# Ensembl/WiggleTools

Hardware: AMD Instinct MI355X
Metric: genomic bp/s (whole node) for 'mean' over N BigWig tracks (higher is better)
Workload: dtype f64

## Files before the change

### wiggletools_amd/csrc/wt_core.h

```cpp
#ifndef WT_CORE_H_
#define WT_CORE_H_

#include <stdint.h>
#include <math.h>
#include <type_traits>

#ifdef WT_EMU
#define WT_DEV inline
#define WT_RESTRICT
#else
#include <hip/hip_runtime.h>
#define WT_DEV __device__ __forceinline__
#define WT_RESTRICT __restrict__
#endif

enum {
    WT_OP_SUM = 0, WT_OP_PRODUCT = 1, WT_OP_MEAN = 2, WT_OP_VAR = 3, WT_OP_STDDEV = 4,
    WT_OP_ENTROPY = 5, WT_OP_CV = 6, WT_OP_MIN = 7, WT_OP_MAX = 8, WT_OP_MEDIAN = 9,
    WT_OP_TTEST = 10, WT_OP_MWU = 11,
    WT_OP_MULTIPLEX = 12
};
#define WT_STRICT_SET0 1u
#define WT_STRICT_SET1 2u

#define WT_FLAG_AGG  (1ull << 62)
#define WT_FLAG_PFX  (2ull << 62)
#define WT_VAL_MASK  ((1ull << 62) - 1)

enum { WT_CTR_TICKET = 0, WT_CTR_RUNS = 1, WT_CTR_BP = 2, WT_CTR_INTERVALS = 3, WT_CTR_ERROR = 4,
       WT_CTR_DELTA_BAD = 5 ,
       WT_CTR_PROF = 8 , WT_CTR_N = 16 };
#define WT_ERR_CAPACITY 1ull
#define WT_ERR_LOOKBACK 2ull

struct WtParams {
    const int32_t *start;
    const int32_t *finish;
    const void *value;
    const int64_t *seg_off;
    const double *defaults;
    int32_t n_chrom, n_tracks;
    long long n_total;
    const int32_t *cbase;
    const int32_t *c_nwin;
    const int32_t *c_hi;
    const int64_t *c_first_win;
    int32_t W;
    int32_t logW;
    int32_t n_words;
    int64_t n_windows;
    const int32_t *win_chrom;
    uint32_t *widx;
    int32_t op;
    uint32_t flags;
    int32_t n_set0;
    int32_t pad0;
    unsigned long long *status;
    unsigned long long *counters;
    unsigned long long *debug;
    int64_t capacity;
    int32_t *o_start;
    int32_t *o_finish;
    double *o_value;
    int64_t *chrom_run_off;
    double *o_tile;
    uint8_t *o_inplay;
    int32_t *bad_list;
    long long *bad_goff;
    char *g_scratch;
    long long g_scratch_slab;
    long long g_attr_slab;
    int32_t chunk_tracks;
    int32_t n_chunks;
    int32_t count_segs;
    int32_t spitch;
    int32_t cpitch;
    int32_t off_S, off_cnt, off_segtot, off_U, off_cover, off_E, off_epfx, off_nextw, off_gbase, off_scratch, off_shared;
    int32_t off_acc, off_ev, off_ltv, off_ltc, off_gtv, off_gtc, off_tbase, off_tpfx, off_tfirst, off_dsh;
    int32_t off_qa, off_ltq, off_gtq;
    int32_t delta_q;
    int32_t off_tdef;
    int32_t delta_df;
    int32_t def_emin, def_emax;
    int32_t off_dflt32;
    int32_t off_wcol, off_wcnt, off_woff, off_wtot, off_wbase, off_wgt, off_wncov, off_wfe, off_wdk, off_wguess;
    int32_t walk_S;
    int32_t walk_capp;
    int32_t walk_ov;
    int32_t walk_pair;
    int32_t walk_off_at;
    int32_t walk_mwu;
    int32_t lds_bytes;
    const double *mwu_table;
    int32_t mwu_kmax;
    int32_t delta_ns;
};

struct WtShared {
    long long ticket;
    long long goffset;
    int32_t chrom, w0, w1, emit_hi;
    long long row;
    int32_t next_bp;
    int32_t n_emit;
    unsigned long long bp_sum;
    unsigned long long n_intervals;
    int32_t bad_slot;
};

template <int K>
struct WtLane {
    double res[K];
};

struct WtCtx {
    uint64_t *SC;
    uint16_t *cnt;
    uint32_t *segtot;
    uint64_t *U;
    uint32_t *cover;
    uint64_t *E;
    uint32_t *epfx;
    int16_t *nextw;
    long long *gbase;
    char *scratch;
    char *attr;
    float *dflt32;
    WtShared *sh;
};

WT_DEV void wt_ctx_init(WtCtx &c, const WtParams &P, char *lds) {
    c.SC = (uint64_t *) (lds + P.off_S);
    c.cnt = (uint16_t *) (lds + P.off_cnt);
    c.segtot = (uint32_t *) (lds + P.off_segtot);
    c.U = (uint64_t *) (lds + P.off_U);
    c.cover = (uint32_t *) (lds + P.off_cover);
    c.E = (uint64_t *) (lds + P.off_E);
    c.epfx = (uint32_t *) (lds + P.off_epfx);
    c.nextw = (int16_t *) (lds + P.off_nextw);
// ... 1459 lines not shown
```

### wiggletools_amd/csrc/wt_delta.h

```cpp
#ifndef WT_DELTA_H_
#define WT_DELTA_H_

#define WT_DELTA_K 8
#define WT_DELTA_GROUP 16
#ifndef WT_DELTA_PARK
#define WT_DELTA_PARK 1
#endif
#ifndef WT_DELTA_U
#define WT_DELTA_U 4
#endif
#define WT_DELTA_TILE (64 * WT_DELTA_U)
#ifndef WT_DELTA_COPY2
#define WT_DELTA_COPY2 1
#endif
#ifndef WT_DELTA_ONE_TILE
#define WT_DELTA_ONE_TILE 1
#endif
#define WT_DELTA_TF 2048
#define WT_MAX_DELTA_T 1024
#define WT_DELTA_SQ_T0 768

struct WtDeltaShared {
    long long base_v;
    int32_t base_c;
// ... 145 lines not shown

WT_DEV int wt_delta_find(const uint32_t *tpfx, int nt, uint32_t jj, int i) {
    int lo = i, hi = nt - 1;
    while (lo < hi) {
        const int mid = (lo + hi) >> 1;
        if (jj >= tpfx[mid + 1]) lo = mid + 1; else hi = mid;
    }
    return lo;
}

template <int U = WT_DELTA_U>
WT_DEV void wt_delta_tile(const WtDeltaCtx &d, int nt, uint32_t M, uint32_t tb, int lane, long long (&g)[U]) {
    const uint32_t tile = tb / (64u * U);
    int i = tile < WT_DELTA_TF ? (int) d.tfirst[tile] : wt_delta_find(d.tpfx, nt, tb, 0);
#pragma unroll
    for (int u = 0; u < U; u++) {
        const uint32_t jj = tb + (uint32_t) lane + 64u * (uint32_t) u;
        g[u] = -1;
        if (jj < M) {
            while (jj >= d.tpfx[i + 1]) i++;
            g[u] = d.tbase[i] + 4ll * (long long) jj;
        }
    }
}

template <int U = WT_DELTA_U>
WT_DEV void wt_delta_pass1(const WtParams &P, WtCtx &c, WtDeltaCtx &d, int tid, int nt) {
    const int wave = tid >> 6, lane = tid & 63, nwaves = nt >> 6;
    const uint32_t *val = (const uint32_t *) P.value;
    const uint32_t M = d.tpfx[nt];
    const uint32_t step = (uint32_t) nwaves * (64u * U);
    int emin = 255, emax = 0, bad = 0;
    uint32_t cur[U], nxt[U];
    uint32_t tb = (uint32_t) wave * (64u * U);
    if (tb < M) {
        long long g[U];
        wt_delta_tile<U>(d, nt, M, tb, lane, g);
#pragma unroll
        for (int u = 0; u < U; u++) cur[u] = g[u] >= 0 ? *(const uint32_t *) ((const char *) val + g[u]) : 0u;
    }
    for (; tb < M; tb += step) {
        if (tb + step < M) {
            long long g[U];
            wt_delta_tile<U>(d, nt, M, tb + step, lane, g);
#pragma unroll
            for (int u = 0; u < U; u++) nxt[u] = g[u] >= 0 ? *(const uint32_t *) ((const char *) val + g[u]) : 0u;
        }
#pragma unroll
        for (int u = 0; u < U; u++) {
            const int e = (int) ((cur[u] >> 23) & 0xffu);
            if (e == 0xff) bad = 1;
            if ((cur[u] & 0x7fffffffu) != 0u) {
                const int ee = e ? e : 1;
                emin = ee < emin ? ee : emin;
                emax = ee > emax ? ee : emax;
            }
        }
#pragma unroll
        for (int u = 0; u < U; u++) cur[u] = nxt[u];
    }
    if (emin <= emax) { wt_lds_min32(&d.dsh->emin, emin); wt_lds_max32(&d.dsh->emax, emax); }
    if (bad) wt_lds_max32(&d.dsh->bad, 1);
}

WT_DEV bool wt_delta_verdict(const WtParams &P, const WtDeltaCtx &d, int &emin) {
    int lo = d.dsh->emin, hi = d.dsh->emax;
    if (lo > hi) { lo = 1; hi = 1; }
    emin = lo;
    return !d.dsh->bad && (hi - lo) <= wt_delta_max_span(P.n_tracks);
}

struct WtDeltaRange {
    uint32_t kmax, kmin;
};

WT_DEV long long wt_delta_scaled(uint32_t vb, int scale) {
    const uint32_t e = (vb >> 23) & 0xffu;
    const uint32_t m = (vb & 0x7fffffu) | ((e < 1u ? e : 1u) << 23);
    const int32_t sgn = (int32_t) vb >> 31;
    const int32_t sm = (int32_t) ((m ^ (uint32_t) sgn) - (uint32_t) sgn);
    return (long long) ((unsigned long long) (long long) sm << (((e > 1u ? e : 1u) - (uint32_t) scale) & 63u));
}

template <bool QQ = false, bool DF = false, bool TT = false>
WT_DEV void wt_delta_apply(WtDeltaCtx &d, WtCtx &c, int32_t w0, uint32_t width, int32_t s, int32_t f, uint32_t vb, uint32_t db,
                           int scale, bool ok, int32_t &my_next, WtDeltaRange &R) {
    const uint32_t key = vb & 0x7fffffffu;
    R.kmax = key > R.kmax ? key : R.kmax;
    R.kmin = key - 1u < R.kmin ? key - 1u : R.kmin;
    long long vi = wt_delta_scaled(vb, scale);
    if (DF) vi -= wt_delta_scaled(db, scale);
    const uint32_t po = TT ? db : 0u;
#ifdef WT_EMU
    if (!ok) vi = 0;
#endif
    const uint32_t cs = (uint32_t) (s - w0), cf = (uint32_t) (f - w0);
    if (cs < width && cf < width) {
        wt_lds_add64((unsigned long long *) &d.acc[po + cs], (unsigned long long) vi);
        wt_lds_add32(&d.ev[po + cs], 1u);
        wt_lds_sub64((unsigned long long *) &d.acc[po + cf], (unsigned long long) vi);
        wt_lds_add32(&d.ev[po + cf], 0x10000u);
        if (QQ && vi) {
            unsigned long long a, b;
            wt_delta_square((unsigned long long) (vi < 0 ? -vi : vi), a, b);
            wt_lds_add64(&d.qa[po + cs], a); wt_lds_add64(&d.qb[po + cs], b);
            wt_lds_sub64(&d.qa[po + cf], a); wt_lds_sub64(&d.qb[po + cf], b);
        }
        return;
    }
    const int32_t w1 = w0 + (int32_t) width;
    if (f == w0) { wt_lds_add32(&d.ev[po], 0x00010001u); return; }
    if (s >= w1) { my_next = s < my_next ? s : my_next; return; }
    unsigned long long qa = 0, qb = 0;
    if (QQ && vi) wt_delta_square((unsigned long long) (vi < 0 ? -vi : vi), qa, qb);
    if (s < w0) {
        const bool second = TT && po != 0u;
        wt_lds_add64((unsigned long long *) (second ? &d.dsh->base_v1 : &d.dsh->base_v), (unsigned long long) vi);
        wt_lds_addi32(second ? &d.dsh->base_c1 : &d.dsh->base_c, 1);
        if (QQ && vi) { wt_lds_add64(second ? &d.dsh->base_qa1 : &d.dsh->base_qa, qa); wt_lds_add64(second ? &d.dsh->base_qb1 : &d.dsh->base_qb, qb); }
    } else {
        if (vi) wt_lds_add64((unsigned long long *) &d.acc[po + cs], (unsigned long long) vi);
        wt_lds_add32(&d.ev[po + cs], 1u);
        if (QQ && vi) { wt_lds_add64(&d.qa[po + cs], qa); wt_lds_add64(&d.qb[po + cs], qb); }
    }
    if (f < w1) {
        if (vi) wt_lds_sub64((unsigned long long *) &d.acc[po + cf], (unsigned long long) vi);
        wt_lds_add32(&d.ev[po + cf], 0x10000u);
        if (QQ && vi) { wt_lds_sub64(&d.qa[po + cf], qa); wt_lds_sub64(&d.qb[po + cf], qb); }
    } else {
        my_next = f < my_next ? f : my_next;
    }
}

template <bool DF>
struct WtDeltaPend {
    unsigned long long mask;
    int32_t s, f;
    uint32_t b;
    uint32_t d[DF ? 1 : 1];
};
#ifdef WT_EMU
WT_DEV unsigned long long wt_delta_ballot(bool c) { return c ? 1ull : 0ull; }
WT_DEV bool wt_delta_in_mask(unsigned long long m, int lane) { return m != 0ull; }
#else
WT_DEV unsigned long long wt_delta_ballot(bool c) { return __builtin_amdgcn_ballot_w64(c); }
WT_DEV bool wt_delta_in_mask(unsigned long long m, int lane) { return (m >> lane) & 1ull; }
#endif
template <bool QQ, bool DF, bool TT = false>
WT_DEV void wt_delta_flush(WtDeltaCtx &d, WtCtx &c, WtDeltaPend<DF || TT> &pn, int lane, int32_t w0, uint32_t width, int scale, bool ok,
                           int32_t &my_next) {
    if (wt_delta_in_mask(pn.mask, lane)) {
        WtDeltaRange scrap;
        scrap.kmax = 0u; scrap.kmin = 0xffffffffu;
        wt_delta_apply<QQ, DF, TT>(d, c, w0, width, pn.s, pn.f, pn.b, (DF || TT) ? pn.d[0] : 0u, scale, ok, my_next, scrap);
    }
    pn.mask = 0ull;
}
template <bool QQ, bool DF, bool TT = false>
WT_DEV void wt_delta_apply_or_park(WtDeltaCtx &d, WtCtx &c, WtDeltaPend<DF || TT> &pn, int lane, bool valid, int32_t w0, uint32_t width,
                                   int32_t s, int32_t f, uint32_t vb, uint32_t db, int scale, bool ok, int32_t &my_next, WtDeltaRange &R) {
    const uint32_t rs = (uint32_t) (s - w0), rf = (uint32_t) (f - w0);
    const bool inside = rs < width && rf < width;
    const uint32_t cs = TT ? rs + db : rs, cf = TT ? rf + db : rf;
    if (valid) {
        const uint32_t key = vb & 0x7fffffffu;
        R.kmax = key > R.kmax ? key : R.kmax;
        R.kmin = key - 1u < R.kmin ? key - 1u : R.kmin;
    }
    if (valid && inside) {
        long long vi = wt_delta_scaled(vb, scale);
        if (DF) vi -= wt_delta_scaled(db, scale);
#ifdef WT_EMU
        if (!ok) vi = 0;
#endif
        wt_lds_add64((unsigned long long *) &d.acc[cs], (unsigned long long) vi);
        wt_lds_add32(&d.ev[cs], 1u);
        wt_lds_sub64((unsigned long long *) &d.acc[cf], (unsigned long long) vi);
        wt_lds_add32(&d.ev[cf], 0x10000u);
        if (QQ && vi) {
            unsigned long long a, b;
            wt_delta_square((unsigned long long) (vi < 0 ? -vi : vi), a, b);
            wt_lds_add64(&d.qa[cs], a); wt_lds_add64(&d.qb[cs], b);
            wt_lds_sub64(&d.qa[cf], a); wt_lds_sub64(&d.qb[cf], b);
        }
    }
    const bool park = valid && !inside;
    const unsigned long long pm = wt_delta_ballot(park);
    if (pm & pn.mask) wt_delta_flush<QQ, DF, TT>(d, c, pn, lane, w0, width, scale, ok, my_next);
    pn.s = park ? s : pn.s;
    pn.f = park ? f : pn.f;
    pn.b = park ? vb : pn.b;
    if (DF || TT) pn.d[0] = park ? db : pn.d[0];
    pn.mask |= pm;
}

template <bool DF, int U = WT_DELTA_U>
struct WtDeltaBatch {
    int32_t s[U], f[U];
    uint32_t b[U];
    uint32_t d[DF ? U : 1];
};

template <bool DF, bool TT = false, int U = WT_DELTA_U>
WT_DEV void wt_delta_fetch(const WtParams &P, const WtDeltaCtx &d, int nt, uint32_t M, uint32_t tb, int lane, WtDeltaBatch<DF || TT, U> &B, int c0 = 0) {
    const uint32_t last = (M - 1u) / (64u * U) * (64u * U);
    const uint32_t tbe = tb < last ? tb : last;
    const uint32_t tile = tbe / (64u * U);
    int i = tile < WT_DELTA_TF ? (int) d.tfirst[tile] : wt_delta_find(d.tpfx, nt, tbe, 0);
    uint32_t hi = d.tpfx[i + 1];
    long long dl = d.tbase[i];
    uint32_t db = DF ? d.tdef[i] : 0u;
    if (TT) db = c0 + i >= P.n_set0 ? (uint32_t) P.W : 0u;
#pragma unroll
    for (int u = 0; u < U; u++) {
        uint32_t jj = tbe + (uint32_t) lane + 64u * (uint32_t) u;
        jj = jj < M - 1u ? jj : M - 1u;
        if (jj >= hi) {
            do { i++; hi = d.tpfx[i + 1]; } while (jj >= hi);
            dl = d.tbase[i];
            if (DF) db = d.tdef[i];
            if (TT) db = c0 + i >= P.n_set0 ? (uint32_t) P.W : 0u;
        }
        const long long ob = dl + ((long long) jj << 2);
        B.s[u] = *(const int32_t *) ((const char *) P.start + ob);
        B.f[u] = *(const int32_t *) ((const char *) P.finish + ob);
        B.b[u] = *(const uint32_t *) ((const char *) P.value + ob);
        if (DF || TT) B.d[u] = db;
    }
}


template <bool QQ = false, bool DF = false, bool TT = false, int U = WT_DELTA_U>
WT_DEV void wt_delta_apply_tile(WtDeltaCtx &d, WtCtx &c, const WtDeltaBatch<DF || TT, U> &B, uint32_t tb, uint32_t M, int lane, int32_t w0,
                                uint32_t width, int scale, bool ok, int32_t &my_next, WtDeltaRange &R, WtDeltaPend<DF || TT> &pn) {
    if constexpr (WT_DELTA_PARK == 2 || (WT_DELTA_PARK == 1 && QQ)) {
        if (tb + (64u * U) <= M) {
#pragma unroll
            for (int u = 0; u < U; u++)
                wt_delta_apply_or_park<QQ, DF, TT>(d, c, pn, lane, true, w0, width, B.s[u], B.f[u], B.b[u], (DF || TT) ? B.d[u] : 0u, scale, ok, my_next, R);
        } else {
#pragma unroll
            for (int u = 0; u < U; u++)
                wt_delta_apply_or_park<QQ, DF, TT>(d, c, pn, lane, tb + (uint32_t) lane + 64u * (uint32_t) u < M, w0, width, B.s[u], B.f[u], B.b[u],
                                               (DF || TT) ? B.d[u] : 0u, scale, ok, my_next, R);
        }
    } else {
        if (tb + (64u * U) <= M) {
#pragma unroll
            for (int u = 0; u < U; u++)
                wt_delta_apply<QQ, DF, TT>(d, c, w0, width, B.s[u], B.f[u], B.b[u], (DF || TT) ? B.d[u] : 0u, scale, ok, my_next, R);
        } else {
#pragma unroll
            for (int u = 0; u < U; u++)
                if (tb + (uint32_t) lane + 64u * (uint32_t) u < M)
                    wt_delta_apply<QQ, DF, TT>(d, c, w0, width, B.s[u], B.f[u], B.b[u], (DF || TT) ? B.d[u] : 0u, scale, ok, my_next, R);
        }
    }
}

template <bool QQ = false, bool DF = false, bool TT = false, int U = WT_DELTA_U>
WT_DEV void wt_delta_pass2(const WtParams &P, WtCtx &c, WtDeltaCtx &d, int scale, bool ok, bool collect, bool stats,
                           int tid, int nt, int ntr = 0, int c0 = 0) {
    const int wave = wt_uniform32(tid >> 6), lane = tid & 63, nwaves = nt >> 6;
    const uint32_t M = (uint32_t) wt_uniform32((int32_t) d.tpfx[nt]);
    const int32_t w0 = wt_uniform32(c.sh->w0);
    const uint32_t width = (uint32_t) (wt_uniform32(c.sh->w1) - w0);
    const uint32_t step = (uint32_t) nwaves * (64u * U);
    int32_t my_next = 0x7fffffff;
    WtDeltaRange R;
    R.kmax = 0u; R.kmin = 0xffffffffu;
    if (DF) {
        unsigned long long dsum = (tid < ntr && ok) ? (unsigned long long) wt_delta_scaled(d.tdef[tid], scale) : 0ull;
        dsum = wt_wave_sum_u64(dsum);
        if (dsum && wt_wave_leader(lane)) wt_lds_add64((unsigned long long *) &d.dsh->base_v, dsum);
    }
    uint32_t tb = (uint32_t) wave * (64u * U);
    if (tb < M) {
        WtDeltaBatch<DF || TT, U> A, B;
        WtDeltaPend<DF || TT> pn;
        pn.mask = 0ull; pn.s = 0; pn.f = 0; pn.b = 0u; pn.d[0] = 0u;
        wt_delta_fetch<DF, TT, U>(P, d, nt, M, tb, lane, A, c0);
#if WT_DELTA_ONE_TILE
        if (tb + step >= M) wt_delta_apply_tile<QQ, DF, TT, U>(d, c, A, tb, M, lane, w0, width, scale, ok, my_next, R, pn);
        else
#endif
        for (;;) {
            wt_delta_fetch<DF, TT, U>(P, d, nt, M, tb + step, lane, B, c0);
            wt_delta_apply_tile<QQ, DF, TT, U>(d, c, A, tb, M, lane, w0, width, scale, ok, my_next, R, pn);
            tb += step;
            if (tb >= M) break;
            wt_delta_fetch<DF, TT, U>(P, d, nt, M, tb + step, lane, A, c0);
            wt_delta_apply_tile<QQ, DF, TT, U>(d, c, B, tb, M, lane, w0, width, scale, ok, my_next, R, pn);
            tb += step;
            if (tb >= M) break;
        }
        if (pn.mask) wt_delta_flush<QQ, DF, TT>(d, c, pn, lane, w0, width, scale, ok, my_next);
    }
    my_next = wt_wave_min_i32(my_next);
    if (my_next != 0x7fffffff && wt_wave_leader(lane)) wt_lds_min32(&c.sh->next_bp, my_next);
    if (collect) {
        const uint32_t kmax = wt_wave_max_u32(R.kmax), kmin = wt_wave_min_u32(R.kmin) + 1u;
        if (kmax != 0u && wt_wave_leader(lane)) {
            const int emax = (int) (kmax >> 23), emin = (int) (kmin >> 23);
            wt_lds_min32(&d.dsh->emin, emin ? emin : 1);
            wt_lds_max32(&d.dsh->emax, emax ? emax : 1);
            if (emax == 0xff) wt_lds_max32(&d.dsh->bad, 1);
        }
    }
    if (stats && tid == 0 && M) wt_lds_add64(&c.sh->n_intervals, (unsigned long long) M);
}

WT_DEV int wt_delta_window_verdict(const WtParams &P, const WtDeltaCtx &d, int guess, int &lo, bool &ok) {
    int a = d.dsh->emin, b = d.dsh->emax;
    const bool bad = d.dsh->bad != 0;
    const int R = wt_delta_max_span(P.n_tracks);
    if (a > b) { lo = guess; ok = !bad; return bad ? 0 : 1; }
    lo = a;
    ok = !bad && (b - a) <= R;
    return (!bad && a >= guess && (b - guess) <= R) ? 1 : 0;
}

WT_DEV void wt_delta_mark_bad(const WtParams &P, WtCtx &c, long long k) {
    const unsigned long long slot = wt_glb_add64(&P.counters[WT_CTR_DELTA_BAD], 1ull);
    c.sh->bad_slot = (int32_t) slot;
    if (P.bad_list) P.bad_list[slot] = (int32_t) k;
}
#define WT_BAD_SUB 16
WT_DEV void wt_delta_note_offset(const WtParams &P, WtCtx &c, int lane) {
    if (c.sh->bad_slot >= 0 && P.bad_goff && lane < WT_BAD_SUB)
        P.bad_goff[(long long) c.sh->bad_slot * WT_BAD_SUB + lane] = c.sh->goffset + (long long) c.epfx[(lane * P.n_words) / WT_BAD_SUB];
}

template <bool QQ = false, bool TT = false>
WT_DEV void wt_delta_rezero(const WtParams &P, WtCtx &c, WtDeltaCtx &d, int tid, int nt) {
    const int np = TT ? 2 * P.W : P.W;
    for (int x = tid; x < np; x += nt) { d.acc[x] = 0; d.ev[x] = 0; }
    if constexpr (QQ)
        for (int x = tid; x < np; x += nt) { d.qa[x] = 0; d.qb[x] = 0; }
    if (tid == 0) {
        d.dsh->base_v = 0; d.dsh->base_c = 0;
        if constexpr (QQ) { d.dsh->base_qa = 0; d.dsh->base_qb = 0; }
        if constexpr (TT) { d.dsh->base_v1 = 0; d.dsh->base_c1 = 0; d.dsh->base_qa1 = 0; d.dsh->base_qb1 = 0; }
    }
}

#ifdef WT_EMU
WT_DEV void wt_lds_load8(const uint32_t *p, uint32_t (&v)[WT_DELTA_K]) { for (int k = 0; k < WT_DELTA_K; k++) v[k] = p[k]; }
WT_DEV void wt_lds_load8(const unsigned long long *p, unsigned long long (&v)[WT_DELTA_K]) { for (int k = 0; k < WT_DELTA_K; k++) v[k] = p[k]; }
#else
WT_DEV void wt_lds_load8(const uint32_t *p, uint32_t (&v)[WT_DELTA_K]) {
    typedef uint32_t wt_u32x4 __attribute__((ext_vector_type(4)));
    const wt_u32x4 a = ((const wt_u32x4 *) p)[0], b = ((const wt_u32x4 *) p)[1];
    v[0] = a.x; v[1] = a.y; v[2] = a.z; v[3] = a.w; v[4] = b.x; v[5] = b.y; v[6] = b.z; v[7] = b.w;
}
WT_DEV void wt_lds_load8(const unsigned long long *p, unsigned long long (&v)[WT_DELTA_K]) {
    typedef unsigned long long wt_u64x2 __attribute__((ext_vector_type(2)));
    const wt_u64x2 a = ((const wt_u64x2 *) p)[0], b = ((const wt_u64x2 *) p)[1], c = ((const wt_u64x2 *) p)[2], e = ((const wt_u64x2 *) p)[3];
    v[0] = a.x; v[1] = a.y; v[2] = b.x; v[3] = b.y; v[4] = c.x; v[5] = c.y; v[6] = e.x; v[7] = e.y;
}
#endif
#ifdef WT_EMU
WT_DEV void wt_lds_load4(const uint32_t *p, uint32_t (&v)[4]) { for (int k = 0; k < 4; k++) v[k] = p[k]; }
WT_DEV void wt_lds_load2(const uint32_t *p, uint32_t (&v)[2]) { v[0] = p[0]; v[1] = p[1]; }
#else
WT_DEV void wt_lds_load4(const uint32_t *p, uint32_t (&v)[4]) {
    typedef uint32_t wt_u32x4 __attribute__((ext_vector_type(4)));
    const wt_u32x4 a = *(const wt_u32x4 *) p;
    v[0] = a.x; v[1] = a.y; v[2] = a.z; v[3] = a.w;
}
WT_DEV void wt_lds_load2(const uint32_t *p, uint32_t (&v)[2]) {
    typedef uint32_t wt_u32x2 __attribute__((ext_vector_type(2)));
    const wt_u32x2 a = *(const wt_u32x2 *) p;
    v[0] = a.x; v[1] = a.y;
}
#endif
WT_DEV void wt_lds_load8(const long long *p, long long (&v)[WT_DELTA_K]) { wt_lds_load8((const unsigned long long *) p, (unsigned long long (&)[WT_DELTA_K]) v); }

template <bool QQ = false>
WT_DEV void wt_delta_scan1(const WtParams &P, WtCtx &c, WtDeltaCtx &d, WtDeltaLane &L, int tid, int nt) {
// ... 122 lines not shown
            unsigned __int128 I;
            if (OP == WT_OP_VAR) I = (unsigned __int128) ((unsigned long long) N * (unsigned long long) N) * Q - (unsigned __int128) (unsigned long long) (2 * N - cov) * s2;
            else I = (unsigned __int128) (unsigned long long) N * Q - s2;
            const double Id = (double) (unsigned long long) (I >> 64) * 18446744073709551616.0 + (double) (unsigned long long) I;
            double r;
            if (OP == WT_OP_VAR) {
                r = Id * q * q / ((double) N * (double) N) / N;
                if (N < 2) r = wt_nan();
            } else {
                r = sqrt(Id * q * q / N / N);
                if (OP == WT_OP_CV) {
                    const double mean = (double) S * q / N;
                    r = mean == 0 ? wt_nan() : r / mean;
                }
            }
            out.res[k] = r;
        }
    }
    ((uint8_t *) c.U)[tid] = (uint8_t) evmask;
    ((uint8_t *) c.E)[tid] = (uint8_t) em;
}

template <bool ISMAX>
WT_DEV void wt_delta_tree_update(uint32_t *tree, uint32_t W, uint32_t l, uint32_t r, uint32_t key) {
    for (l += W, r += W; l < r; l >>= 1, r >>= 1) {
        if (l & 1u) { if (ISMAX) wt_lds_umax32(&tree[l], key); else wt_lds_umin32(&tree[l], key); l++; }
        if (r & 1u) { --r; if (ISMAX) wt_lds_umax32(&tree[r], key); else wt_lds_umin32(&tree[r], key); }
    }
}

template <bool ISMAX>
WT_DEV void wt_delta_zero_mm(const WtParams &P, WtCtx &c, WtDeltaCtx &d, int tid, int nt) {
    uint32_t *tree = (uint32_t *) d.acc;
    const uint32_t none = ISMAX ? 0u : 0xffffffffu;
    for (int x = tid; x < 2 * P.W; x += nt) tree[x] = none;
    for (int x = tid; x < P.W; x += nt) d.ev[x] = 0;
    if (tid == 0) { d.dsh->base_v = 0; d.dsh->base_c = 0; d.dsh->emin = 255; d.dsh->emax = 0; d.dsh->bad = 0; }
}

template <bool ISMAX>
WT_DEV void wt_delta_apply_mm(WtDeltaCtx &d, WtCtx &c, int32_t w0, uint32_t width, int32_t s, int32_t f, uint32_t vb, int32_t &my_next, bool &bad) {
    bad |= (vb & 0x7fffffffu) > 0x7f800000u || vb == 0x80000000u;
    const uint32_t key = wt_key32(__builtin_bit_cast(float, vb));
    const uint32_t cs = (uint32_t) (s - w0), cf = (uint32_t) (f - w0);
    uint32_t l, r;
    if (cs < width && cf < width) {
        wt_lds_add32(&d.ev[cs], 1u);
        wt_lds_add32(&d.ev[cf], 0x10000u);
        l = cs; r = cf;
    } else {
        const int32_t w1 = w0 + (int32_t) width;
        if (f == w0) { wt_lds_add32(&d.ev[0], 0x00010001u); return; }
        if (s >= w1) { my_next = s < my_next ? s : my_next; return; }
        if (s < w0) { wt_lds_addi32(&d.dsh->base_c, 1); l = 0u; }
        else { wt_lds_add32(&d.ev[cs], 1u); l = cs; }
        if (f < w1) { wt_lds_add32(&d.ev[cf], 0x10000u); r = cf; }
        else { my_next = f < my_next ? f : my_next; r = width; }
    }
    wt_delta_tree_update<ISMAX>((uint32_t *) d.acc, width, l, r, key);
}

template <bool ISMAX>
WT_DEV void wt_delta_pass_mm(const WtParams &P, WtCtx &c, WtDeltaCtx &d, int tid, int nt) {
    const int wave = wt_uniform32(tid >> 6), lane = tid & 63, nwaves = nt >> 6;
    const uint32_t M = (uint32_t) wt_uniform32((int32_t) d.tpfx[nt]);
    const int32_t w0 = wt_uniform32(c.sh->w0);
    const uint32_t width = (uint32_t) (wt_uniform32(c.sh->w1) - w0);
    const uint32_t step = (uint32_t) nwaves * WT_DELTA_TILE;
    int32_t my_next = 0x7fffffff;
    bool bad = false;
    uint32_t tb = (uint32_t) wave * WT_DELTA_TILE;
    if (tb < M) {
        WtDeltaBatch<false> A, B;
        auto apply = [&](const WtDeltaBatch<false> &T, uint32_t at) {
            if (at + WT_DELTA_TILE <= M) {
#pragma unroll
                for (int u = 0; u < WT_DELTA_U; u++) wt_delta_apply_mm<ISMAX>(d, c, w0, width, T.s[u], T.f[u], T.b[u], my_next, bad);
            } else {
#pragma unroll
                for (int u = 0; u < WT_DELTA_U; u++)
                    if (at + (uint32_t) lane + 64u * (uint32_t) u < M) wt_delta_apply_mm<ISMAX>(d, c, w0, width, T.s[u], T.f[u], T.b[u], my_next, bad);
            }
        };
        wt_delta_fetch<false>(P, d, nt, M, tb, lane, A);
#if WT_DELTA_ONE_TILE
        if (tb + step >= M) apply(A, tb);
        else
#endif
        for (;;) {
            wt_delta_fetch<false>(P, d, nt, M, tb + step, lane, B);
            apply(A, tb);
            tb += step;
            if (tb >= M) break;
            wt_delta_fetch<false>(P, d, nt, M, tb + step, lane, A);
            apply(B, tb);
            tb += step;
            if (tb >= M) break;
        }
    }
    my_next = wt_wave_min_i32(my_next);
    if (my_next != 0x7fffffff && wt_wave_leader(lane)) wt_lds_min32(&c.sh->next_bp, my_next);
    if (wt_delta_ballot(bad) != 0ull && wt_wave_leader(lane)) wt_lds_max32(&d.dsh->bad, 1);
    if (tid == 0 && M) wt_lds_add64(&c.sh->n_intervals, (unsigned long long) M);
}

WT_DEV void wt_delta_scan1_mm(const WtParams &P, WtCtx &c, WtDeltaCtx &d, int32_t &tc, int tid, int nt) {
    const int p0 = tid * WT_DELTA_K;
    int32_t rc = 0;
    uint32_t e8[WT_DELTA_K];
    wt_lds_load8(d.ev + p0, e8);
#pragma unroll
    for (int k = 0; k < WT_DELTA_K; k++) {
        const uint32_t e = e8[k];
        rc += (int32_t) (e & 0xffffu) - (int32_t) (e >> 16);
    }
    tc = rc;
    d.ltc[tid] = rc;
}
WT_DEV void wt_delta_scan2_mm(const WtParams &P, WtCtx &c, WtDeltaCtx &d, int tid, int nt) {
    const int ngroups = nt / WT_DELTA_GROUP;
    if (tid >= ngroups) return;
    int32_t sc = 0;
    for (int x = 0; x < WT_DELTA_GROUP; x++) sc += d.ltc[tid * WT_DELTA_GROUP + x];
    d.gtc[tid] = sc;
}

template <bool ISMAX>
WT_DEV void wt_delta_scan3_mm(const WtParams &P, WtCtx &c, WtDeltaCtx &d, int32_t wc, WtLane<WT_DELTA_K> &out, int tid, int nt) {
    int32_t bc = d.dsh->base_c;
#ifdef WT_EMU
    const int grp = tid / WT_DELTA_GROUP;
    for (int x = 0; x < grp; x++) bc += d.gtc[x];
    for (int x = grp * WT_DELTA_GROUP; x < tid; x++) bc += d.ltc[x];
#else
    bc += (int32_t) wt_waves_before32((const uint32_t *) d.gtc, 0, tid >> 6, tid & 63);
    bc += wc;
#endif
    const int N = P.n_tracks;
    const bool strict = (P.flags & WT_STRICT_SET0) != 0;
    const int p0 = tid * WT_DELTA_K;
    const long long room = (long long) c.sh->emit_hi - ((long long) c.sh->w0 + p0);
    const uint32_t *tree = (const uint32_t *) d.acc;
    const uint32_t W = (uint32_t) P.W;
    auto best = [](uint32_t a, uint32_t b) { return ISMAX ? (a > b ? a : b) : (a < b ? a : b); };
    uint32_t top = ISMAX ? 0u : 0xffffffffu;
    for (uint32_t n = ((uint32_t) p0 + W) >> 3; n >= 1u; n >>= 1) top = best(top, tree[n]);
    uint32_t em = 0, evmask = 0;
    uint32_t e8[WT_DELTA_K];
    wt_lds_load8(d.ev + p0, e8);
    uint32_t lf[WT_DELTA_K], par[4], gp[2];
    wt_lds_load8(tree + W + (uint32_t) p0, lf);
    wt_lds_load4(tree + ((W + (uint32_t) p0) >> 1), par);
    wt_lds_load2(tree + ((W + (uint32_t) p0) >> 2), gp);
#pragma unroll
    for (int k = 0; k < WT_DELTA_K; k++) {
        const uint32_t e = e8[k];
        bc += (int32_t) (e & 0xffffu) - (int32_t) (e >> 16);
        evmask |= (e != 0u ? 1u : 0u) << k;
        const bool pred = strict ? (bc == N) : (bc > 0);
        if (e != 0u && pred && k < room) em |= 1u << k;
        const uint32_t key = best(best(lf[k], par[k >> 1]), best(gp[k >> 2], top));
        double v = (double) wt_unkey32(key);
        if (bc < N) v = ISMAX ? (v < 0.0 ? 0.0 : v) : (v > 0.0 ? 0.0 : v);
        out.res[k] = v;
    }
    ((uint8_t *) c.U)[tid] = (uint8_t) evmask;
    ((uint8_t *) c.E)[tid] = (uint8_t) em;
}

struct WtDeltaLane2 {
    long long tv;
    int32_t tc;
    unsigned long long tqa, tqb;
    long long wv;
    int32_t wc;
    unsigned long long wqa, wqb;
};
// ... 388 lines not shown
```

### wiggletools_amd/csrc/wt_engine.hip

```cpp
#include <hip/hip_runtime.h>

#include <cstdio>
#include <thread>
#include <atomic>
#include <cstring>
#include <map>
#include <mutex>
#include <string>
#include <vector>

#include "wt_host.h"
#include "wt_trackset.h"
#include "wt_core.h"
#include "wt_plan.h"
#include "wt_kernels.h"
#include "wt_devscope.h"
#include "wt_pool.h"

#ifndef WT_INDEX_UNROLL
#define WT_INDEX_UNROLL 2
#endif
#define WT_INDEX_CHUNK (256 * 4 * WT_INDEX_UNROLL)
__global__ void __launch_bounds__(256) wt_index_kernel(const WtParams P, long long total, long long span) {
    const long long dev_total = P.seg_off[(long long) P.n_chrom * P.n_tracks];
// ... 744 lines not shown
            }
            return rc;
        }
        if (rc != WTAMD_OK && rc != WTAMD_ERR_CAPACITY) return rc;
        const long long n_bad = (long long) ts->h_counters[WT_CTR_DELTA_BAD];
        if (n_bad == 0) { ts->delta_verified_[dc] = true; ts->delta_n_bad_[dc] = 0; return rc; }
        if (wt_few_enough_to_patch(n_bad, ts->stats.n_windows) && !getenv("WTAMD_NO_PATCH")) {
            const int rp = wt_launch_patch(ts, plan.W, op, flags, n_set0, runs, n_bad, s);
            if (rp == WTAMD_OK) {
                WT_HIP(hipStreamSynchronize(s));
                ts->delta_verified_[dc] = true;
                ts->delta_n_bad_[dc] = n_bad;
                return rc;
            }
            if (rp != WTAMD_ERR_INTERNAL) return rp;
        }
        ts->delta_failed_[dc] = true;
    }
    if (!wt_pick_plan(ts, op, n_set0, plan, err, s)) return wt_fail(WTAMD_ERR_ARG, err);
    return wt_reduce_plan(ts, plan, op, flags, n_set0, runs, d_tile, d_inplay, n_runs, s);
}

extern "C++" int wt_reduce_enqueue(wtamd_trackset *ts, const wtamd_reduce_desc &desc, wtamd_runs *runs, double *d_tile, uint8_t *d_inplay,
                                   hipStream_t s, bool *used_delta, int *delta_W) {
    WtPlan plan;
    std::string err;
    *used_delta = !d_tile && wt_wants_delta(ts, desc.op);
    if (*used_delta) {
        wt_make_delta_plan_for(plan, ts->n_tracks, desc.op);
        *delta_W = plan.W;
    } else if (!wt_pick_plan(ts, desc.op, desc.n_set0, plan, err, s)) {
        return wt_fail(WTAMD_ERR_ARG, err);
    }
    return wt_reduce_plan(ts, plan, desc.op, desc.flags, desc.n_set0, runs, d_tile, d_inplay, nullptr, s);
}

static int wt_reduce_plan(wtamd_trackset *ts, const WtPlan &plan, int op, uint32_t flags, int n_set0, wtamd_runs *runs,
                          double *d_tile, uint8_t *d_inplay, int64_t *n_runs, hipStream_t s) {
    if (plan.T > (plan.delta ? ((wt_op_is_var_family(op) || op == WT_OP_TTEST) ? wt_delta_sq_block : wt_delta_block) : wt_reduce_max_block)) return wt_fail(WTAMD_ERR_ARG, "workgroup size above the kernel's launch bound");
    WtWindows *w = nullptr;
    int rc = wt_get_windows(ts, plan.W, &w, s);
    if (rc != WTAMD_OK) return rc;
    if (!w->indexed) {
        rc = wt_build_index(ts, w, plan, s);
        if (rc != WTAMD_OK) return rc;
    }
    WtLaunch L;
    wt_fill_params(ts, w, plan, L.P);
    L.P.op = op; L.P.flags = flags; L.P.n_set0 = n_set0;
    L.P.capacity = runs->capacity;
    L.P.o_start = runs->start; L.P.o_finish = runs->finish; L.P.o_value = runs->value;
    L.P.chrom_run_off = runs->chrom_run_off ? runs->chrom_run_off : ts->d_chrom_run_off;
    L.P.o_tile = d_tile; L.P.o_inplay = d_inplay;
    L.T = plan.T; L.lds = plan.lds_bytes; L.stream = s; L.num_cu = ts->num_cu;
    L.gscratch = &ts->d_gscratch; L.gscratch_bytes = &ts->gscratch_bytes;
    if (op == WT_OP_MWU && !getenv("WTAMD_MWU_DEVICE_ERF")) {
        const int n1 = n_set0, n2 = ts->n_tracks - n_set0;
        if (ts->mwu_n1 != n1 || ts->mwu_n2 != n2) {
            std::vector<double> t;
            const bool have = wt_mwu_make_table(n1, n2, t);
            if (ts->d_mwu_table) { ts->mwu_retired.push_back(ts->d_mwu_table); ts->d_mwu_table = nullptr; }
            if (have) {
                WT_HIP(hipMalloc((void **) &ts->d_mwu_table, sizeof(double) * t.size()));
                WT_HIP(hipMemcpyAsync(ts->d_mwu_table, t.data(), sizeof(double) * t.size(), hipMemcpyHostToDevice, s));
                WT_HIP(hipStreamSynchronize(s));
            }
            ts->mwu_n1 = n1; ts->mwu_n2 = n2; ts->mwu_kmax = have ? (int) t.size() - 1 : 0;
        }
        L.P.mwu_table = ts->d_mwu_table;
        L.P.mwu_kmax = ts->mwu_kmax;
    }
    if (plan.delta) {
        const int64_t nwin = w->tab.n_windows > 0 ? w->tab.n_windows : 1;
        if (w->cap_bad < nwin) {
            int64_t c1 = w->cap_bad, c2 = w->cap_bad;
            bool quiet = false;
            WT_HIP(wt_grow(&w->d_bad_list, &c1, nwin, &quiet));
            WT_HIP(wt_grow(&w->d_bad_goff, &c2, nwin * WT_BAD_SUB, &quiet));
            w->cap_bad = c1 < c2 / WT_BAD_SUB ? c1 : c2 / WT_BAD_SUB;
        }
        L.P.bad_list = w->d_bad_list;
        L.P.bad_goff = w->d_bad_goff;
        wt_delta_defaults_params(ts->defaults.data(), ts->n_tracks, L.P);
    }

    const bool launches = w->tab.n_windows > 0 && ts->n_intervals > 0;
    {
        const long long n_status = launches ? (long long) w->tab.n_windows : 0;
        const long long most = std::max<long long>(std::max<long long>(n_status, WT_CTR_N), ts->n_chrom + 1);
        const unsigned blocks = (unsigned) std::min<long long>((most + 255) / 256, 1024);
        hipLaunchKernelGGL(wt_clear_kernel, dim3(blocks), dim3(256), 0, s, ts->d_counters, (int) WT_CTR_N, L.P.chrom_run_off, ts->n_chrom + 1,
                           w->d_status, n_status);
        WT_HIP(hipGetLastError());
    }
    if (launches) {
        if (plan.delta) {
            static const int force_u = getenv("WTAMD_DELTA_U") ? atoi(getenv("WTAMD_DELTA_U")) : 0;
            const double tiles_per_wave = (double) ts->n_intervals / (double) w->tab.n_windows / 256.0 / (double) std::max(1, L.T / 64);
            L.small_tiles = force_u == 2 || (force_u != 4 && tiles_per_wave < 8.0);
        }
        WT_HIP(hipEventRecord(ts->ev_r0, s));
        if (plan.delta) {
            wt_delta_launch(L, op);
        } else if (plan.walk_S) {
            L.err = wt_walk_launch(L.P, plan.regcol, L.T, L.lds, L.num_cu, L.gscratch, L.gscratch_bytes, L.stream, &L.grid);
        } else if (!wt_reduce_launch(L, op, ts->value_f64, ts->scratch_f32, plan.ppt, plan.n_chunks > 1 || plan.scratch_slab > 0, plan.regcol)) {
            return wt_fail(WTAMD_ERR_ARG, "op not dispatchable");
        }
        if (L.err != hipSuccess) return wt_fail(WTAMD_ERR_HIP, std::string("kernel launch: ") + hipGetErrorString(L.err));
        WT_HIP(hipEventRecord(ts->ev_r1, s));
        ts->have_reduce_time = true;
    }
    ts->stats.n_windows = w->tab.n_windows;
    ts->stats.window_bp = plan.W;
    ts->stats.lds_bytes = plan.lds_bytes;
    ts->stats.kernel = plan.delta ? 1 : (plan.walk_S ? (plan.walk_mwu ? 3 : 2) : 0);
    ts->stats.patched_windows = 0;
    if (n_runs) {
        WT_HIP(hipMemcpyAsync(ts->h_counters, ts->d_counters, sizeof(unsigned long long) * WT_CTR_N, hipMemcpyDeviceToHost, s));
        const int rcw = wt_bounded_wait([s] { return hipStreamQuery(s); }, "hipStreamQuery", nullptr, 0.002, 200, [ts](double limit_s) {
            char buf[320];
            snprintf(buf, sizeof buf, "kernel did not finish within %.0f s (debug marker %llu, window %lld; per wave %llu %llu %llu %llu %llu %llu %llu %llu)",
                     limit_s, ts->h_debug[0], (long long) ts->h_debug[1], ts->h_debug[2], ts->h_debug[3], ts->h_debug[4],
                     ts->h_debug[5], ts->h_debug[6], ts->h_debug[7], ts->h_debug[8], ts->h_debug[9]);
            return std::string(buf);
        });
        if (rcw != WTAMD_OK) return rcw;
        ts->stats.n_runs = (int64_t) ts->h_counters[WT_CTR_RUNS];
        ts->stats.covered_bp = (int64_t) ts->h_counters[WT_CTR_BP];
        ts->stats.n_intervals = (int64_t) ts->h_counters[WT_CTR_INTERVALS];
        *n_runs = ts->stats.n_runs;
        if (plan.walk_S) {
            static const bool show = getenv("WTAMD_WALK_PROF") != nullptr;
            if (show) {
                static const char *names_w[8] = {"zero+ranges", "count", "offsets", "scatter", "events", "first-median", "moves", "rest"};
                unsigned long long tot = 0;
                for (int q = 0; q < 8; q++) tot += ts->h_counters[WT_CTR_PROF + q];
                fprintf(stderr, "[wt_walk_profile]");
                for (int q = 0; q < 8; q++) fprintf(stderr, " %s %.1f%%", names_w[q], tot ? 100.0 * ts->h_counters[WT_CTR_PROF + q] / tot : 0.0);
                fprintf(stderr, " (total %.3g cycles)\n", (double) tot);
            }
        }
#ifdef WT_PROFILE
        {
            static const char *names_g[8] = {"zero", "load", "count", "emask+escan", "eval", "lookback", "write", "-"};
            static const char *names_d[8] = {"zero", "ranges", "pass1", "pass2", "scan", "escan", "lookback", "write"};
            const char **names = plan.delta ? names_d : names_g;
            unsigned long long tot = 0;
            for (int q = 0; q < 8; q++) tot += ts->h_counters[WT_CTR_PROF + q];
            fprintf(stderr, "[wt_profile] op %d:", op);
            for (int q = 0; q < 8; q++)
                fprintf(stderr, " %s %.1f%%", names[q], tot ? 100.0 * ts->h_counters[WT_CTR_PROF + q] / tot : 0.0);
            fprintf(stderr, " (total %.3g cycles over all workgroups)\n", (double) tot);
            unsigned long long p2[8] = {0};
            if (wt_prof2_take(p2))
                fprintf(stderr, "[wt_profile] register column, cycles summed over waves: gather %.3g  sort/park %.3g  count loop %.3g  erf %.3g  median sort+select %.3g\n",
                        (double) p2[0], (double) p2[1], (double) p2[2], (double) p2[3], (double) p2[4]);
        }
#endif
        if (ts->h_counters[WT_CTR_ERROR] & WT_ERR_LOOKBACK) return wt_fail(WTAMD_ERR_INTERNAL, "look-back timed out");
        if (ts->h_counters[WT_CTR_ERROR] & WT_ERR_CAPACITY) return wt_fail(WTAMD_ERR_CAPACITY, "output capacity too small");
    }
    return WTAMD_OK;
}

int wtamd_reduce(wtamd_trackset *ts, const wtamd_reduce_desc *desc, wtamd_runs *runs, int64_t *n_runs, void *stream) {
    int rc = wt_check_desc(ts, desc);
    if (rc != WTAMD_OK) return rc;
    return wt_reduce_impl(ts, desc->op, desc->flags, desc->n_set0, runs, nullptr, nullptr, n_runs, (hipStream_t) stream);
}

static int wt_reduce_host_impl(wtamd_trackset *ts, int op, uint32_t flags, int n_set0, wtamd_runs *runs,
                               double *h_tile, uint8_t *h_inplay, int64_t *n_runs) {
    if (!runs) return wt_fail(WTAMD_ERR_ARG, "runs == NULL");
    int64_t cap = wtamd_trackset_max_runs(ts);
    if (cap > runs->capacity) cap = runs->capacity;
    const int64_t alloc = cap > 0 ? cap : 1;
    const int N = ts->n_tracks;
    WtDevScope scope;
    wtamd_runs d{};
// ... 149 lines not shown
```

Baseline: 50.76 billion.

## Use 32-bit per-lane offsets from a uniform base for delta tile fetches

Delta-path tile fetches now compute one wave-uniform 64-bit base and give each lane a 32-bit offset. This lets loads use scalar-base plus vector-offset addressing instead of full 64-bit per-lane address arithmetic. If the tile's span exceeds 4GB, or an env flag forces it, the tile is refetched with the old 64-bit path. A magic-number float-to-fixed conversion is also added, but it is compiled out by default (WT_DELTA_MAGIC=0).

```diff
diff --git a/wiggletools_amd/csrc/wt_core.h b/wiggletools_amd/csrc/wt_core.h
--- a/wiggletools_amd/csrc/wt_core.h
+++ b/wiggletools_amd/csrc/wt_core.h
@@ -54,7 +54,7 @@
     int32_t op;
     uint32_t flags;
     int32_t n_set0;
-    int32_t pad0;
+    int32_t delta_addr64;
     unsigned long long *status;
     unsigned long long *counters;
     unsigned long long *debug;
diff --git a/wiggletools_amd/csrc/wt_delta.h b/wiggletools_amd/csrc/wt_delta.h
--- a/wiggletools_amd/csrc/wt_delta.h
+++ b/wiggletools_amd/csrc/wt_delta.h
@@ -251,14 +251,56 @@
     return (long long) ((unsigned long long) (long long) sm << (((e > 1u ? e : 1u) - (uint32_t) scale) & 63u));
 }
 
-template <bool QQ = false, bool DF = false, bool TT = false>
+#ifndef WT_DELTA_MAGIC
+#define WT_DELTA_MAGIC 0
+#endif
+#define WT_DELTA_MAGIC_SPAN 26
+WT_DEV bool wt_delta_magic_fits(int n_tracks) { return wt_delta_max_span(n_tracks) <= WT_DELTA_MAGIC_SPAN; }
+WT_DEV bool wt_delta_magic_route(int n_tracks) { return WT_DELTA_MAGIC && wt_delta_magic_fits(n_tracks); }
+WT_DEV unsigned long long wt_delta_magic_bits(int scale) {
+    return ((unsigned long long) (1023 + 52 - 150 + scale) << 52) | (1ull << 51);
+}
+WT_DEV unsigned long long wt_delta_magic_sum(uint32_t vb, unsigned long long magic) {
+    return __builtin_bit_cast(unsigned long long, (double) __builtin_bit_cast(float, vb) + __builtin_bit_cast(double, magic));
+}
+WT_DEV long long wt_delta_scaled_magic(uint32_t vb, unsigned long long magic) {
+    const unsigned long long sum = wt_delta_magic_sum(vb, magic);
+    uint32_t hi = (uint32_t) (sum >> 32) - (uint32_t) (magic >> 32);
+#ifndef WT_EMU
+    asm("" : "+v"(hi));
+#endif
+    return (long long) (((unsigned long long) hi << 32) | (sum & 0xffffffffull));
+}
+
+struct WtDeltaUnit {
+    int scale;
+    unsigned long long magic;
+};
+WT_DEV WtDeltaUnit wt_delta_unit(int scale) {
+    WtDeltaUnit un;
+    un.scale = scale;
+    un.magic = wt_delta_magic_bits(scale);
+    return un;
+}
+template <bool MG, bool DF>
+WT_DEV long long wt_delta_units(uint32_t vb, uint32_t db, const WtDeltaUnit &un) {
+    if constexpr (MG) {
+        if constexpr (DF) return (long long) (wt_delta_magic_sum(vb, un.magic) - wt_delta_magic_sum(db, un.magic));
+        else return wt_delta_scaled_magic(vb, un.magic);
+    } else {
+        long long vi = wt_delta_scaled(vb, un.scale);
+        if constexpr (DF) vi -= wt_delta_scaled(db, un.scale);
+        return vi;
+    }
+}
+
+template <bool QQ = false, bool DF = false, bool TT = false, bool MG = false>
 WT_DEV void wt_delta_apply(WtDeltaCtx &d, WtCtx &c, int32_t w0, uint32_t width, int32_t s, int32_t f, uint32_t vb, uint32_t db,
-                           int scale, bool ok, int32_t &my_next, WtDeltaRange &R) {
+                           const WtDeltaUnit &un, bool ok, int32_t &my_next, WtDeltaRange &R) {
     const uint32_t key = vb & 0x7fffffffu;
     R.kmax = key > R.kmax ? key : R.kmax;
     R.kmin = key - 1u < R.kmin ? key - 1u : R.kmin;
-    long long vi = wt_delta_scaled(vb, scale);
-    if (DF) vi -= wt_delta_scaled(db, scale);
+    long long vi = wt_delta_units<MG, DF>(vb, db, un);
     const uint32_t po = TT ? db : 0u;
 #ifdef WT_EMU
     if (!ok) vi = 0;
@@ -315,19 +357,19 @@
 WT_DEV unsigned long long wt_delta_ballot(bool c) { return __builtin_amdgcn_ballot_w64(c); }
 WT_DEV bool wt_delta_in_mask(unsigned long long m, int lane) { return (m >> lane) & 1ull; }
 #endif
-template <bool QQ, bool DF, bool TT = false>
-WT_DEV void wt_delta_flush(WtDeltaCtx &d, WtCtx &c, WtDeltaPend<DF || TT> &pn, int lane, int32_t w0, uint32_t width, int scale, bool ok,
+template <bool QQ, bool DF, bool TT = false, bool MG = false>
+WT_DEV void wt_delta_flush(WtDeltaCtx &d, WtCtx &c, WtDeltaPend<DF || TT> &pn, int lane, int32_t w0, uint32_t width, const WtDeltaUnit &un, bool ok,
                            int32_t &my_next) {
     if (wt_delta_in_mask(pn.mask, lane)) {
         WtDeltaRange scrap;
         scrap.kmax = 0u; scrap.kmin = 0xffffffffu;
-        wt_delta_apply<QQ, DF, TT>(d, c, w0, width, pn.s, pn.f, pn.b, (DF || TT) ? pn.d[0] : 0u, scale, ok, my_next, scrap);
+        wt_delta_apply<QQ, DF, TT, MG>(d, c, w0, width, pn.s, pn.f, pn.b, (DF || TT) ? pn.d[0] : 0u, un, ok, my_next, scrap);
     }
     pn.mask = 0ull;
 }
-template <bool QQ, bool DF, bool TT = false>
+template <bool QQ, bool DF, bool TT = false, bool MG = false>
 WT_DEV void wt_delta_apply_or_park(WtDeltaCtx &d, WtCtx &c, WtDeltaPend<DF || TT> &pn, int lane, bool valid, int32_t w0, uint32_t width,
-                                   int32_t s, int32_t f, uint32_t vb, uint32_t db, int scale, bool ok, int32_t &my_next, WtDeltaRange &R) {
+                                   int32_t s, int32_t f, uint32_t vb, uint32_t db, const WtDeltaUnit &un, bool ok, int32_t &my_next, WtDeltaRange &R) {
     const uint32_t rs = (uint32_t) (s - w0), rf = (uint32_t) (f - w0);
     const bool inside = rs < width && rf < width;
     const uint32_t cs = TT ? rs + db : rs, cf = TT ? rf + db : rf;
@@ -337,8 +379,7 @@
         R.kmin = key - 1u < R.kmin ? key - 1u : R.kmin;
     }
     if (valid && inside) {
-        long long vi = wt_delta_scaled(vb, scale);
-        if (DF) vi -= wt_delta_scaled(db, scale);
+        long long vi = wt_delta_units<MG, DF>(vb, db, un);
 #ifdef WT_EMU
         if (!ok) vi = 0;
 #endif
@@ -355,7 +396,7 @@
     }
     const bool park = valid && !inside;
     const unsigned long long pm = wt_delta_ballot(park);
-    if (pm & pn.mask) wt_delta_flush<QQ, DF, TT>(d, c, pn, lane, w0, width, scale, ok, my_next);
+    if (pm & pn.mask) wt_delta_flush<QQ, DF, TT, MG>(d, c, pn, lane, w0, width, un, ok, my_next);
     pn.s = park ? s : pn.s;
     pn.f = park ? f : pn.f;
     pn.b = park ? vb : pn.b;
@@ -368,10 +409,11 @@
     int32_t s[U], f[U];
     uint32_t b[U];
     uint32_t d[DF ? U : 1];
+    bool near;
 };
 
 template <bool DF, bool TT = false, int U = WT_DELTA_U>
-WT_DEV void wt_delta_fetch(const WtParams &P, const WtDeltaCtx &d, int nt, uint32_t M, uint32_t tb, int lane, WtDeltaBatch<DF || TT, U> &B, int c0 = 0) {
+WT_DEV void wt_delta_fetch64(const WtParams &P, const WtDeltaCtx &d, int nt, uint32_t M, uint32_t tb, int lane, WtDeltaBatch<DF || TT, U> &B, int c0 = 0) {
     const uint32_t last = (M - 1u) / (64u * U) * (64u * U);
     const uint32_t tbe = tb < last ? tb : last;
     const uint32_t tile = tbe / (64u * U);
@@ -396,33 +438,95 @@
         B.b[u] = *(const uint32_t *) ((const char *) P.value + ob);
         if (DF || TT) B.d[u] = db;
     }
-}
-
-
-template <bool QQ = false, bool DF = false, bool TT = false, int U = WT_DELTA_U>
+    B.near = true;
+}
+
+#ifndef WT_DELTA_SADDR
+#define WT_DELTA_SADDR 1
+#endif
+WT_DEV bool wt_delta_near(long long top) { return (unsigned long long) top < (1ull << 32); }
+WT_DEV uint32_t wt_delta_off32(long long dd, uint32_t jr) { return (uint32_t) (unsigned long long) dd + (jr << 2); }
+#ifdef WT_EMU
+WT_DEV long long wt_delta_lane63(long long x) { return x; }
+#else
+WT_DEV long long wt_delta_lane63(long long x) {
+    const unsigned lo = (unsigned) __builtin_amdgcn_readlane((int) (unsigned) (unsigned long long) x, 63);
+    const unsigned hi = (unsigned) __builtin_amdgcn_readlane((int) (unsigned) ((unsigned long long) x >> 32), 63);
+    return (long long) (((unsigned long long) hi << 32) | lo);
+}
+#endif
+template <bool DF, bool TT = false, int U = WT_DELTA_U>
+WT_DEV void wt_delta_fetch(const WtParams &P, const WtDeltaCtx &d, int nt, uint32_t M, uint32_t tb, int lane, WtDeltaBatch<DF || TT, U> &B, int c0 = 0) {
+    const uint32_t last = (M - 1u) / (64u * U) * (64u * U);
+    const uint32_t tbe = tb < last ? tb : last;
+    const uint32_t tile = tbe / (64u * U);
+    const uint32_t jmax = M - 1u - tbe;
+    const uint32_t jtop = 64u * U - 1u < jmax ? 64u * U - 1u : jmax;
+    int i = wt_uniform32(tile < WT_DELTA_TF ? (int) d.tfirst[tile] : wt_delta_find(d.tpfx, nt, tbe, 0));
+    uint32_t hi = d.tpfx[i + 1];
+    const long long dl0 = wt_uniform64(d.tbase[i]);
+    const long long base = dl0 + ((long long) tbe << 2);
+    long long dd = 0;
+    uint32_t db = DF ? d.tdef[i] : 0u;
+    if (TT) db = c0 + i >= P.n_set0 ? (uint32_t) P.W : 0u;
+    uint32_t off[U];
+#pragma unroll
+    for (int u = 0; u < U; u++) {
+        uint32_t jr = (uint32_t) lane + 64u * (uint32_t) u;
+        jr = jr < jmax ? jr : jmax;
+        if (tbe + jr >= hi) {
+            do { i++; hi = d.tpfx[i + 1]; } while (tbe + jr >= hi);
+            dd = d.tbase[i] - dl0;
+            if (DF) db = d.tdef[i];
+            if (TT) db = c0 + i >= P.n_set0 ? (uint32_t) P.W : 0u;
+        }
+        off[u] = wt_delta_off32(dd, jr);
+        if (DF || TT) B.d[u] = db;
+    }
+#ifdef WT_EMU
+    const long long top = d.tbase[wt_delta_find(d.tpfx, nt, tbe + jtop, i)] - dl0 + ((long long) jtop << 2);
+#else
+    const long long top = wt_delta_lane63(dd) + ((long long) jtop << 2);
+#endif
+    B.near = wt_delta_near(top) && !P.delta_addr64;
+    const char *ps = (const char *) P.start + base, *pf = (const char *) P.finish + base, *pv = (const char *) P.value + base;
+#pragma unroll
+    for (int u = 0; u < U; u++) {
+        B.s[u] = *(const int32_t *) (ps + off[u]);
+        B.f[u] = *(const int32_t *) (pf + off[u]);
+        B.b[u] = *(const uint32_t *) (pv + off[u]);
+    }
+}
+template <bool DF, bool TT = false, int U = WT_DELTA_U>
+WT_DEV void wt_delta_refetch(const WtParams &P, const WtDeltaCtx &d, int nt, uint32_t M, uint32_t tb, int lane, WtDeltaBatch<DF || TT, U> &B, int c0 = 0) {
+    if (!B.near) wt_delta_fetch64<DF, TT, U>(P, d, nt, M, tb, lane, B, c0);
+}
+
+
+template <bool QQ = false, bool DF = false, bool TT = false, int U = WT_DELTA_U, bool MG = false>
 WT_DEV void wt_delta_apply_tile(WtDeltaCtx &d, WtCtx &c, const WtDeltaBatch<DF || TT, U> &B, uint32_t tb, uint32_t M, int lane, int32_t w0,
-                                uint32_t width, int scale, bool ok, int32_t &my_next, WtDeltaRange &R, WtDeltaPend<DF || TT> &pn) {
+                                uint32_t width, const WtDeltaUnit &un, bool ok, int32_t &my_next, WtDeltaRange &R, WtDeltaPend<DF || TT> &pn) {
     if constexpr (WT_DELTA_PARK == 2 || (WT_DELTA_PARK == 1 && QQ)) {
         if (tb + (64u * U) <= M) {
 #pragma unroll
             for (int u = 0; u < U; u++)
-                wt_delta_apply_or_park<QQ, DF, TT>(d, c, pn, lane, true, w0, width, B.s[u], B.f[u], B.b[u], (DF || TT) ? B.d[u] : 0u, scale, ok, my_next, R);
+                wt_delta_apply_or_park<QQ, DF, TT, MG>(d, c, pn, lane, true, w0, width, B.s[u], B.f[u], B.b[u], (DF || TT) ? B.d[u] : 0u, un, ok, my_next, R);
         } else {
 #pragma unroll
             for (int u = 0; u < U; u++)
-                wt_delta_apply_or_park<QQ, DF, TT>(d, c, pn, lane, tb + (uint32_t) lane + 64u * (uint32_t) u < M, w0, width, B.s[u], B.f[u], B.b[u],
-                                               (DF || TT) ? B.d[u] : 0u, scale, ok, my_next, R);
+                wt_delta_apply_or_park<QQ, DF, TT, MG>(d, c, pn, lane, tb + (uint32_t) lane + 64u * (uint32_t) u < M, w0, width, B.s[u], B.f[u], B.b[u],
+                                               (DF || TT) ? B.d[u] : 0u, un, ok, my_next, R);
         }
     } else {
         if (tb + (64u * U) <= M) {
 #pragma unroll
             for (int u = 0; u < U; u++)
-                wt_delta_apply<QQ, DF, TT>(d, c, w0, width, B.s[u], B.f[u], B.b[u], (DF || TT) ? B.d[u] : 0u, scale, ok, my_next, R);
+                wt_delta_apply<QQ, DF, TT, MG>(d, c, w0, width, B.s[u], B.f[u], B.b[u], (DF || TT) ? B.d[u] : 0u, un, ok, my_next, R);
         } else {
 #pragma unroll
             for (int u = 0; u < U; u++)
                 if (tb + (uint32_t) lane + 64u * (uint32_t) u < M)
-                    wt_delta_apply<QQ, DF, TT>(d, c, w0, width, B.s[u], B.f[u], B.b[u], (DF || TT) ? B.d[u] : 0u, scale, ok, my_next, R);
+                    wt_delta_apply<QQ, DF, TT, MG>(d, c, w0, width, B.s[u], B.f[u], B.b[u], (DF || TT) ? B.d[u] : 0u, un, ok, my_next, R);
         }
     }
 }
@@ -438,8 +542,11 @@
     int32_t my_next = 0x7fffffff;
     WtDeltaRange R;
     R.kmax = 0u; R.kmin = 0xffffffffu;
+    const WtDeltaUnit un = wt_delta_unit(wt_uniform32(scale));
+    const bool mg = !QQ && wt_delta_magic_route(P.n_tracks);
     if (DF) {
-        unsigned long long dsum = (tid < ntr && ok) ? (unsigned long long) wt_delta_scaled(d.tdef[tid], scale) : 0ull;
+        unsigned long long dsum = 0ull;
+        if (tid < ntr && ok) dsum = (unsigned long long) (mg ? wt_delta_scaled_magic(d.tdef[tid], un.magic) : wt_delta_scaled(d.tdef[tid], un.scale));
         dsum = wt_wave_sum_u64(dsum);
         if (dsum && wt_wave_leader(lane)) wt_lds_add64((unsigned long long *) &d.dsh->base_v, dsum);
     }
@@ -448,22 +555,35 @@
         WtDeltaBatch<DF || TT, U> A, B;
         WtDeltaPend<DF || TT> pn;
         pn.mask = 0ull; pn.s = 0; pn.f = 0; pn.b = 0u; pn.d[0] = 0u;
-        wt_delta_fetch<DF, TT, U>(P, d, nt, M, tb, lane, A, c0);
+        constexpr bool NEAR = WT_DELTA_SADDR && !QQ && U == WT_DELTA_U;
+        auto fetch = [&](WtDeltaBatch<DF || TT, U> &T, uint32_t at) {
+            if constexpr (NEAR) wt_delta_fetch<DF, TT, U>(P, d, nt, M, at, lane, T, c0);
+            else wt_delta_fetch64<DF, TT, U>(P, d, nt, M, at, lane, T, c0);
+        };
+        auto apply = [&](WtDeltaBatch<DF || TT, U> &T, uint32_t at) {
+            if constexpr (NEAR) wt_delta_refetch<DF, TT, U>(P, d, nt, M, at, lane, T, c0);
+            if (mg) wt_delta_apply_tile<QQ, DF, TT, U, true>(d, c, T, at, M, lane, w0, width, un, ok, my_next, R, pn);
+            else wt_delta_apply_tile<QQ, DF, TT, U, false>(d, c, T, at, M, lane, w0, width, un, ok, my_next, R, pn);
+        };
+        fetch(A, tb);
 #if WT_DELTA_ONE_TILE
-        if (tb + step >= M) wt_delta_apply_tile<QQ, DF, TT, U>(d, c, A, tb, M, lane, w0, width, scale, ok, my_next, R, pn);
+        if (tb + step >= M) apply(A, tb);
         else
 #endif
         for (;;) {
-            wt_delta_fetch<DF, TT, U>(P, d, nt, M, tb + step, lane, B, c0);
-            wt_delta_apply_tile<QQ, DF, TT, U>(d, c, A, tb, M, lane, w0, width, scale, ok, my_next, R, pn);
+            fetch(B, tb + step);
+            apply(A, tb);
             tb += step;
             if (tb >= M) break;
-            wt_delta_fetch<DF, TT, U>(P, d, nt, M, tb + step, lane, A, c0);
-            wt_delta_apply_tile<QQ, DF, TT, U>(d, c, B, tb, M, lane, w0, width, scale, ok, my_next, R, pn);
+            fetch(A, tb + step);
+            apply(B, tb);
             tb += step;
             if (tb >= M) break;
         }
-        if (pn.mask) wt_delta_flush<QQ, DF, TT>(d, c, pn, lane, w0, width, scale, ok, my_next);
+        if (pn.mask) {
+            if (mg) wt_delta_flush<QQ, DF, TT, true>(d, c, pn, lane, w0, width, un, ok, my_next);
+            else wt_delta_flush<QQ, DF, TT, false>(d, c, pn, lane, w0, width, un, ok, my_next);
+        }
     }
     my_next = wt_wave_min_i32(my_next);
     if (my_next != 0x7fffffff && wt_wave_leader(lane)) wt_lds_min32(&c.sh->next_bp, my_next);
@@ -752,17 +872,17 @@
                     if (at + (uint32_t) lane + 64u * (uint32_t) u < M) wt_delta_apply_mm<ISMAX>(d, c, w0, width, T.s[u], T.f[u], T.b[u], my_next, bad);
             }
         };
-        wt_delta_fetch<false>(P, d, nt, M, tb, lane, A);
+        wt_delta_fetch64<false>(P, d, nt, M, tb, lane, A);
 #if WT_DELTA_ONE_TILE
         if (tb + step >= M) apply(A, tb);
         else
 #endif
         for (;;) {
-            wt_delta_fetch<false>(P, d, nt, M, tb + step, lane, B);
+            wt_delta_fetch64<false>(P, d, nt, M, tb + step, lane, B);
             apply(A, tb);
             tb += step;
             if (tb >= M) break;
-            wt_delta_fetch<false>(P, d, nt, M, tb + step, lane, A);
+            wt_delta_fetch64<false>(P, d, nt, M, tb + step, lane, A);
             apply(B, tb);
             tb += step;
             if (tb >= M) break;
diff --git a/wiggletools_amd/csrc/wt_engine.hip b/wiggletools_amd/csrc/wt_engine.hip
--- a/wiggletools_amd/csrc/wt_engine.hip
+++ b/wiggletools_amd/csrc/wt_engine.hip
@@ -850,6 +850,8 @@
         L.P.bad_list = w->d_bad_list;
         L.P.bad_goff = w->d_bad_goff;
         wt_delta_defaults_params(ts->defaults.data(), ts->n_tracks, L.P);
+        const char *e64 = getenv("WTAMD_DELTA_ADDR64");
+        L.P.delta_addr64 = (e64 && atoi(e64)) ? 1 : 0;
     }
 
     const bool launches = w->tab.n_windows > 0 && ts->n_intervals > 0;
@@ -863,7 +865,8 @@
     }
     if (launches) {
         if (plan.delta) {
-            static const int force_u = getenv("WTAMD_DELTA_U") ? atoi(getenv("WTAMD_DELTA_U")) : 0;
+            const char *eU = getenv("WTAMD_DELTA_U");
+            const int force_u = eU ? atoi(eU) : 0;
             const double tiles_per_wave = (double) ts->n_intervals / (double) w->tab.n_windows / 256.0 / (double) std::max(1, L.T / 64);
             L.small_tiles = force_u == 2 || (force_u != 4 && tiles_per_wave < 8.0);
         }
```

Result: no change. 50.32 billion (-0.9%).
